# vita-epfl/collaborative-gan-sampling

Hardware: AMD Instinct MI355X
Metric: refined samples/sec @ 20 refinement steps (higher is better)
Workload: dtype f32; 1 GPU; dcgan64 collaborative refinement (propose + K-step refine + render), batch 1024/GPU, K=20, momentum rate 0.1, refine at feature [8, 8, 256], random-init weights, z~U(-1,1) seed 2019+rank; global_batch=1024, refine_steps=20, parallelism=single GPU, hipgraph=True, batches_in_flight=2, fused_per_launch=1, sync_bn=False, contraction=f32

## Files before the change

### collaborative-gan-sampling_amd/csrc/bn.hip

```cpp
#include "cgs_internal.h"

#define BN_MAX_BLOCKS CGS_BN_MAX_BLOCKS

struct BnGeom {
    int G;
    int rows_per_block;
};

static BnGeom bn_geom(int M, int C) {
    BnGeom g;
    int rpb = cgs_ceil_div(M, BN_MAX_BLOCKS);
    if (rpb < 16) rpb = 16;
    g.rows_per_block = rpb;
    g.G = cgs_ceil_div(M, rpb);
    (void)C;
    return g;
}

size_t cgs_bn_ws_bytes(int M, int C) {
    (void)M;
    return ((size_t)BN_MAX_BLOCKS * 2 * C + 6 * (size_t)C) * sizeof(float);
}

__device__ __forceinline__ void bn_affine4(const float* __restrict__ mean, const float* __restrict__ invstd, const float* __restrict__ gamma,
// ... 695 lines not shown
                                     const float* gamma, const float* beta, const float* mean, const float* invstd, float leak, float* dx,
                                     int M_group, int C, void* ws, size_t ws_bytes, void* stream) {
    if (groups <= 0 || groups > 65535 || M_group <= 0 || C <= 0 || (C & 3) || rows_per_seg <= 0 || nseg <= 0 || seg_stride < 0 || !part || !dy || !x || !dx)
        return cgs_set_error(CGS_EINVAL, "norm bwd from partials: groups=%d M=%d C=%d rows=%d x %d", groups, M_group, C, rows_per_seg, nseg);
    const bool sliced = groups == 1 && nseg == 1 && rows_per_seg >= 1024 && !((uintptr_t)ws & 7);
    const size_t need = (size_t)groups * 2 * C * sizeof(float) + (sliced ? (size_t)BNF_SLICES * 2 * C * sizeof(double) : 0);
    if (!ws || ws_bytes < need) return cgs_set_error(CGS_EWORKSPACE, "norm bwd from partials: workspace %zu < %zu", ws_bytes, need);
    hipStream_t s = (hipStream_t)stream;
    if (const int rpb = norm_fa_rows_per_block(groups, rows_per_seg, nseg, M_group, C)) {
        hipLaunchKernelGGL(norm_fa_kernel<true>, dim3(cgs_ceil_div(C, 64), cgs_ceil_div(M_group, rpb), groups), dim3(256), 0, s, x, dy, part, rows_per_seg, nseg,
                           seg_stride, gamma, beta, 0.f, leak, dx, (float*)mean, (float*)invstd, M_group, C, rpb);
        CGS_CHECK_LAUNCH("norm_lrelu_bwd_from_partials");
        return CGS_OK;
    }
    float* stat2;
    if (sliced) {
        double* slices = (double*)ws;
        stat2 = (float*)(slices + (size_t)BNF_SLICES * 2 * C);
        hipLaunchKernelGGL(bn_slice_sums_kernel, dim3(cgs_ceil_div(C, BNF_CH), BNF_SLICES), dim3(256), 0, s, part, rows_per_seg, C, slices);
        hipLaunchKernelGGL(bn_finalize2_slices_kernel, dim3(cgs_ceil_div(C, 64)), dim3(64), 0, s, slices, M_group, C, stat2);
    } else {
        stat2 = (float*)ws;
        hipLaunchKernelGGL(bn_finalize_kernel<1>, dim3(cgs_ceil_div(C, BNF_CH), groups), dim3(256), 0, s, part, rows_per_seg, M_group, C, nullptr, nullptr, 0.f,
                           stat2, nullptr, nullptr, nseg, seg_stride);
    }
    const size_t n4 = (size_t)groups * M_group * C / 4, gn4 = (size_t)M_group * C / 4;
    hipLaunchKernelGGL(bn_apply_bwd_kernel, dim3(ew_blocks(n4)), dim3(256), 0, s, dy, x, mean, invstd, gamma, beta, stat2, leak, dx, n4, C, gn4);
    CGS_CHECK_LAUNCH("norm_lrelu_bwd_from_partials");
    return CGS_OK;
}

int cgs_instnorm_lrelu_bwd_data(const float* dy, const float* x, const float* scale, const float* offset, const float* mean,
                                const float* invstd, float leak, float* dx, int B, int HW, int C, void* ws, size_t ws_bytes,
                                void* stream) {
    if (B <= 0 || HW <= 0 || C <= 0 || (C & 3) || B > 65535) return cgs_set_error(CGS_EINVAL, "instnorm bwd: B=%d HW=%d C=%d", B, HW, C);
    if (ws_bytes < cgs_instnorm_ws_bytes(B, HW, C)) return cgs_set_error(CGS_EWORKSPACE, "instnorm bwd: workspace %zu < %zu", ws_bytes, cgs_instnorm_ws_bytes(B, HW, C));
    hipStream_t s = (hipStream_t)stream;
    const BnGeom g = in_geom(B, HW);
    float* part = (float*)ws;
    float* stat = part + (size_t)B * g.G * 2 * C;
    float* stat2 = stat + (size_t)B * 4 * C;
    if (norm_small_ok(HW)) {
        hipLaunchKernelGGL(norm_small_kernel<true>, dim3(cgs_ceil_div(C, 64), B), dim3(256), 0, s, x, dy, scale, offset, 0.f, leak, dx, (float*)mean, (float*)invstd, stat2, HW, C);
        CGS_CHECK_LAUNCH("instnorm_lrelu_bwd_data");
        return CGS_OK;
    }
    hipLaunchKernelGGL(bn_partial_kernel<1>, dim3(g.G, B), dim3(256), 0, s, x, dy, mean, invstd, scale, offset, leak, part, HW, C, g.rows_per_block);
    hipLaunchKernelGGL(bn_finalize_kernel<1>, dim3(cgs_ceil_div(C, BNF_CH), B), dim3(256), 0, s, part, g.G, HW, C, nullptr, nullptr, 0.f, stat2, nullptr, nullptr);
    const size_t n4 = (size_t)B * HW * C / 4, gn4 = (size_t)HW * C / 4;
    hipLaunchKernelGGL(bn_apply_bwd_kernel, dim3(ew_blocks(n4)), dim3(256), 0, s, dy, x, mean, invstd, scale, offset, stat2, leak, dx, n4, C, gn4);
    CGS_CHECK_LAUNCH("instnorm_lrelu_bwd_data");
    return CGS_OK;
}
```

### collaborative-gan-sampling_amd/engine.py

```python
import gc

import numpy as np
import torch

from . import kernels as K
from . import lib as L
from .nets import ARCHS, _same_out, g_input_shape, layer_ks


class _Stage:
    out = None
    bwd_epi = (L.EPI_NONE, None, None)
    pre_folded = False
    bwd_nstat = None
    bstat = None

    def fwd(self, x):
        raise NotImplementedError

    def bwd(self, dy):
        raise NotImplementedError


class _View(_Stage):
# ... 47 lines not shown
            elif self.epi == L.EPI_TANH:
                dy = K.tanh_bwd(dy, self.out, out=dy)
        e, a, aux = self.bwd_epi
        return K.conv2d_bwd_data(dy, self.w, self.in_hw, self.s, self.s, out=self.dx, epilogue=e, ep_a=a, ep_aux=aux, nstat=self.bwd_nstat)


class _Deconv(_Stage):

    def __init__(self, B, in_shape, out_shape, w, b, stride, epi, a, c, dev):
        self.w, self.b, self.s, self.epi, self.a, self.c = w, b, stride, epi, a, c
        self.in_hw, self.out_hw = (in_shape[0], in_shape[1]), (out_shape[0], out_shape[1])
        self.out = torch.empty((B,) + tuple(out_shape), dtype=torch.float32, device=dev)
        self.dx = torch.empty((B,) + tuple(in_shape), dtype=torch.float32, device=dev)

    signs = None
    bwd_signs = None
    part = None
    part_layout = None

    def want_stats(self, B, group_images=None):
        if self.epi != L.EPI_NONE:
            return None
        lay = K.conv_stat_layout(L.DECONV_FWD, *self.call_dims(), self.s, self.s, group_images or B)
        if lay is not None:
            self.part = torch.empty((lay[0], 2, self.w.shape[2]), dtype=torch.float32, device=self.out.device)
            self.part_layout = lay
        return self.part

    def fwd(self, x):
        return K.deconv2d_fwd(x, self.w, self.b, self.out_hw, self.s, self.s, self.epi, self.a, self.c, out=self.out, signs=self.signs,
                              part=self.part)

    def bwd(self, dy):
        if not self.pre_folded:
            if self.epi == L.EPI_AFFINE_RELU:
                dy = K.affine_relu_bwd(dy, self.out, self.a, out=dy)
            elif self.epi == L.EPI_TANH:
                dy = K.tanh_bwd(dy, self.out, out=dy)
        e, a, aux = self.bwd_epi
        return K.deconv2d_bwd_data(dy, self.w, self.in_hw, self.s, self.s, out=self.dx, epilogue=e, ep_a=a, ep_aux=aux,
                                   ep_signs=self.bwd_signs, nstat=self.bwd_nstat)

    def call_dims(self):
        kh, kw, Cout, Cin = self.w.shape
        return (self.out.shape[0], self.in_hw[0], self.in_hw[1], Cin, self.out_hw[0], self.out_hw[1], Cout, kh, kw)


class _Linear(_Stage):
    def __init__(self, B, w, b, epi, dev):
        self.w, self.b, self.epi = w, b, epi
        self.out = torch.empty((B, w.shape[1]), dtype=torch.float32, device=dev)
        self.dx = torch.empty((B, w.shape[0]), dtype=torch.float32, device=dev)

    def fwd(self, x):
        self.x_in = x
        return K.linear_fwd(x, self.w, self.b, self.epi, out=self.out)

    def bwd(self, dy):
        if self.epi == L.EPI_LRELU:
            dy = K.lrelu_bwd(dy, self.out, out=dy)
        return K.linear_bwd_data(dy, self.w, out=self.dx)


class _BnTrainLrelu(_Stage):

    def __init__(self, B, shape, gamma, beta, leak, dev):
        self.gamma, self.beta, self.leak = gamma, beta, leak
        self.out = torch.empty((B,) + tuple(shape), dtype=torch.float32, device=dev)
        self.mean = torch.empty(shape[-1], dtype=torch.float32, device=dev)
        self.invstd = torch.empty(shape[-1], dtype=torch.float32, device=dev)
        self.x = None

    sync = None
    groups = 1
    part = None

    part_layout = None

    def set_groups(self, groups, producer=None):
        self.groups = int(groups)
        self.part = self.part_layout = None
        if producer is not None:
            producer.part = producer.part_layout = None
            B = self.out.shape[0]
            self.part = producer.want_stats(B, B // self.groups)
            self.part_layout = producer.part_layout
        C = self.out.shape[-1]
        self.mean = torch.empty((self.groups, C), dtype=torch.float32, device=self.out.device)
        self.invstd = torch.empty((self.groups, C), dtype=torch.float32, device=self.out.device)

    def _g(self, t):
        return t.view(self.groups, -1, t.shape[-1])

    def fwd(self, x):
        self.x = x
        if self.bstat is not None:
            self.bstat.x = x
        if self.groups > 1:
            if self.part is not None:
                K.groupnorm_lrelu_fwd_from_partials(x, self.part, self.part_layout, self.groups, self.gamma, self.beta, self.leak,
                                                    out=self.out, stats=(self.mean, self.invstd))
            else:
                K.instnorm_lrelu_fwd(self._g(x), self.gamma, self.beta, self.leak, out=self._g(self.out), stats=(self.mean, self.invstd))
            return self.out
        if self.sync is None:
            if self.part is not None:
                K.bn_train_lrelu_fwd_from_partials(x, self.part, self.gamma, self.beta, self.leak, out=self.out, stats=(self.mean, self.invstd))
            else:
                K.bn_train_lrelu_fwd(x, self.gamma, self.beta, self.leak, out=self.out, stats=(self.mean, self.invstd))
            return self.out
        M = x.numel() // x.shape[-1]
        sums = self.sync.sums(x.shape[-1], x.device)
        K.bn_sync_fwd_sums(x, sums)
        self.sync.all_reduce(sums)
        K.bn_sync_fwd_apply(x, self.gamma, self.beta, sums, self.sync.world * M, self.leak, out=self.out,
                            stats=(self.mean, self.invstd))
        return self.out

    def bwd(self, dy):
        if self.bstat is not None:
            return K.norm_lrelu_bwd_from_partials(dy, self.x, self.bstat, self.groups, out=dy)
        if self.groups > 1:
            K.instnorm_lrelu_bwd_data(self._g(dy), self._g(self.x), self.gamma, self.beta, self.mean, self.invstd, self.leak,
                                      out=self._g(dy))
            return dy
        if self.sync is None:
            return K.bn_train_lrelu_bwd_data(dy, self.x, self.gamma, self.beta, self.mean, self.invstd, self.leak, out=dy)
        M = self.x.numel() // self.x.shape[-1]
        sums = self.sync.sums(self.x.shape[-1], dy.device)
        K.bn_sync_bwd_sums(dy, self.x, self.gamma, self.beta, self.mean, self.invstd, sums, self.leak)
        self.sync.all_reduce(sums)
        return K.bn_sync_bwd_apply(dy, self.x, self.gamma, self.beta, self.mean, self.invstd, sums, self.sync.world * M,
                                   self.leak, out=dy)


class BnSync:

    def __init__(self, group=None):
        import torch.distributed as dist
        if not (dist.is_available() and dist.is_initialized()):
            raise L.CgsError("sync_bn needs an initialised torch.distributed process group")
        self.dist, self.group = dist, group
        self.world = dist.get_world_size(group)
        self.on_device = dist.get_backend(group) == "nccl"
        self._sums = {}

    def sums(self, C, dev):
        key = (C, dev)
        if key not in self._sums:
            self._sums[key] = torch.empty((2, C), dtype=torch.float64, device=dev)
        return self._sums[key]

    def all_reduce(self, sums):
        if self.world == 1:
            return
        if self.on_device:
            self.dist.all_reduce(sums, group=self.group)
        else:
            h = sums.cpu()
            self.dist.all_reduce(h, group=self.group)
            sums.copy_(h)


class _InstNormAct(_Stage):

    def __init__(self, B, shape, scale, offset, leak, dev):
        self.scale, self.offset, self.leak = scale, offset, leak
        self.out = torch.empty((B,) + tuple(shape), dtype=torch.float32, device=dev)
        self.mean = torch.empty((B, shape[-1]), dtype=torch.float32, device=dev)
        self.invstd = torch.empty((B, shape[-1]), dtype=torch.float32, device=dev)
        self.x = None

# ... 123 lines not shown
            else:
                if kind(i + 1) != "relu":
                    raise NotImplementedError("inference-mode bn is only supported when followed by relu")
                a, c = fold(Lr[1])
                stages.append(_AffineRelu(B, shape, a, c, dev)); i += 2
        elif t == "instnorm":
            sc = f"{scope}/{Lr[1]}"
            leak, used = (K.LEAK, 2) if kind(i + 1) == "lrelu" else (0.0, 2) if kind(i + 1) == "relu" else (1.0, 1)
            in_stage = _InstNormAct(B, shape, P[sc + "/scale"], P[sc + "/offset"], leak, dev)
            if stages and isinstance(stages[-1], (_Conv, _Deconv)):
                in_stage.part = stages[-1].want_stats(B, 1)
                in_stage.part_layout = stages[-1].part_layout
            stages.append(in_stage); i += used
        elif t == "res":
            inner, ishape = compile_layers(Lr[1], shape, P, scope, B, k, stride, bn_training, dev, folds)
            assert tuple(ishape) == tuple(shape)
            stages.append(_Residual(B, shape, inner, dev)); i += 1
        elif t in ("relu", "lrelu", "tanh"):
            stages.append(_Unary(B, shape, t, dev)); i += 1
        elif t == "reshape":
            stages.append(_View((B,) + shape, (B,) + tuple(Lr[1]))); shape = tuple(Lr[1]); i += 1
        elif t == "flatten":
            flat = (int(np.prod(shape)),)
            stages.append(_View((B,) + shape, (B,) + flat)); shape = flat; i += 1
        else:
            raise KeyError(t)
    return stages, shape


def link_backward_fusion(stages):
    for below, above in zip(stages[:-1], stages[1:]):
        if not isinstance(above, (_Conv, _Deconv)) or below.pre_folded:
            continue
        if isinstance(below, _Deconv) and below.epi == L.EPI_AFFINE_RELU:
            above.bwd_epi = (L.EPI_RELU_BWD_AFFINE, below.a, below.out)
            import os
            if isinstance(above, _Deconv) and not os.environ.get("CGS_NO_SIGN_MASKS"):
                s_ = (below.s, below.s)
                if (K.conv_signs_ok(L.DECONV_FWD, *below.call_dims(), *s_, L.EPI_AFFINE_RELU)
                        and K.conv_signs_ok(L.DECONV_BWD_DATA, *above.call_dims(), above.s, above.s, L.EPI_RELU_BWD_AFFINE)):
                    below.signs = torch.empty(below.out.numel() // 32, dtype=torch.int32, device=below.out.device)
                    above.bwd_signs = below.signs
        elif isinstance(below, _Deconv) and below.epi == L.EPI_TANH:
            above.bwd_epi = (L.EPI_TANH_BWD, None, below.out)
        elif isinstance(below, _Conv) and below.epi == L.EPI_LRELU:
            above.bwd_epi = (L.EPI_LRELU_BWD, None, below.out)
        elif isinstance(below, _Conv) and below.epi == L.EPI_TANH:
            above.bwd_epi = (L.EPI_TANH_BWD, None, below.out)
        else:
            continue
        below.pre_folded = True


NSTAT_MAX_BYTES = 48 * 2 ** 20


def link_norm_backward_stats(stages, B):
    for below, above in zip(stages[:-1], stages[1:]):
        if isinstance(below, _Residual):
            link_norm_backward_stats(below.inner, B)
        if not isinstance(above, (_Conv, _Deconv)) or above.bwd_epi[0] != L.EPI_NONE or above.bwd_nstat is not None:
            continue
        if isinstance(below, _BnTrainLrelu) and below.sync is None:
            gamma, beta, gimg = below.gamma, below.beta, B // below.groups
        elif isinstance(below, _InstNormAct):
            gamma, beta, gimg = below.scale, below.offset, 1
        else:
            continue
        C = below.out.shape[-1]
        if below.out.numel() * 4 > NSTAT_MAX_BYTES:
            continue
        if isinstance(above, _Conv):
            H, W, Cin = above.dx.shape[1:]
            kh, kw, _, Cout = above.w.shape
            lay = K.conv_stat_layout(L.CONV_BWD_DATA, B, H, W, Cin, 0, 0, Cout, kh, kw, above.s, above.s, gimg)
        else:
            lay = K.conv_stat_layout(L.DECONV_BWD_DATA, *above.call_dims(), above.s, above.s, gimg)
        if lay is None:
            continue
        part = torch.empty((lay[0], 2, C), dtype=torch.float32, device=below.out.device)
        below.bstat = above.bwd_nstat = K.NormBwdStats(None, below.mean, below.invstd, gamma, beta, below.leak, gimg, part, lay)
    if stages and isinstance(stages[-1], _Residual):
        link_norm_backward_stats(stages[-1].inner, B)


class Tape:

    def __init__(self, layers, in_shape, P, scope, B, k, stride, bn_training, dev):
        self.folds = []
        self.stages, self.out_shape = compile_layers(layers, in_shape, P, scope, B, k, stride, bn_training, dev, self.folds)

    def forward(self, x):
        for st in self.stages:
            x = st.fwd(x)
        return x

    def backward(self, dy):
        for st in reversed(self.stages):
            dy = st.bwd(dy)
        return dy


def _entry(fn):
    import functools

    @functools.wraps(fn)
    def wrapped(self, *a, **kw):
        prev = K.set_contraction(self.contraction)
        try:
            return fn(self, *a, **kw)
        finally:
            if prev != self.contraction:
                K.set_contraction(prev)
    return wrapped


class RefineEngine:

    def __init__(self, arch, params, batch_size, device=None, use_graph=False, sync_bn=None, bn_groups=1, contraction="f32"):
        self.A = ARCHS[arch] if isinstance(arch, str) else arch
        if contraction not in L.CONTRACTIONS:
            raise L.CgsError(f"contraction {contraction!r}: expected one of {sorted(L.CONTRACTIONS)}")
        self.contraction = contraction
        self.dev = torch.device(device if device is not None else "cuda:0")
        if self.dev.type != "cuda":
            raise L.CgsError("RefineEngine needs a GPU device (there is no CPU path)")
        L.load()
        prev_mode = K.set_contraction(self.contraction)
        try:
            self._build(params, batch_size, use_graph, sync_bn, bn_groups)
        finally:
            if prev_mode != self.contraction:
                K.set_contraction(prev_mode)

    def _build(self, params, batch_size, use_graph, sync_bn, bn_groups):
        A, B = self.A, int(batch_size)
        self.B, self.P = B, params
        with torch.cuda.device(self.dev):
            self.g_head = Tape(A["g_head"], g_input_shape(A), params, "generator", B, A["k"], A["stride"], False, self.dev)
            self.g_tail = Tape(A["g_tail"], A["feature"], params, "generator", B, A["k"], A["stride"], False, self.dev)
            self.d = Tape(A["d"], A["img"], params, "discriminator", B, A["k"], A["stride"], True, self.dev)
            link_backward_fusion(self.g_tail.stages + self.d.stages)
            fs = (B,) + tuple(A["feature"])
            f32 = dict(dtype=torch.float32, device=self.dev)
            self.theta, self.mom, self.best_theta = torch.empty(fs, **f32), torch.empty(fs, **f32), torch.empty(fs, **f32)
            self.logit, self.best_logit = torch.empty(B, **f32), torch.empty(B, **f32)
            self.default_logit, self.best_step = torch.empty(B, **f32), torch.empty(B, **f32)
            self.tickets = torch.zeros(B, dtype=torch.int32, device=self.dev)
            self.dlogits = torch.empty((B,) + tuple(self.d.out_shape), **f32)
            self.forced = torch.zeros(B, dtype=torch.int32, device=self.dev)
            self.images = torch.empty((B,) + tuple(A["img"]), **f32)
        self.use_graph = use_graph
        self._graphs = {}
        self._gstream = None
        self._ws_epoch = K.WS.epoch
        self.bn_groups = int(bn_groups)
        if self.bn_groups > 1:
            if B % self.bn_groups:
                raise L.CgsError(f"bn_groups={bn_groups} does not divide the engine batch {B}")
            if sync_bn:
                raise L.CgsError("bn_groups and sync_bn are mutually exclusive")

            def walk_g(stages):
                for below, st in zip([None] + stages[:-1], stages):
                    if isinstance(st, _BnTrainLrelu):
                        st.set_groups(self.bn_groups, below if isinstance(below, _Conv) else None)
                    if isinstance(st, _Residual):
                        walk_g(st.inner)
            walk_g(self.d.stages); walk_g(self.g_tail.stages)
        self.sync_bn = None
        if sync_bn is not None and sync_bn is not False:
            if use_graph:
                raise L.CgsError("sync_bn runs eagerly: the all-reduce between the two halves of a bn pass is not captured")
            self.sync_bn = BnSync(None if sync_bn is True else sync_bn)

            def walk(stages):
                for st in stages:
                    if isinstance(st, _BnTrainLrelu):
                        st.sync = self.sync_bn
                    if isinstance(st, _Residual):
                        walk(st.inner)
            walk(self.d.stages); walk(self.g_tail.stages)

        def drop_partials(stages):
            for below, st in zip([None] + stages[:-1], stages):
                if isinstance(st, _BnTrainLrelu) and st.sync is not None:
                    st.part = None
                    if isinstance(below, _Conv):
                        below.part = None
                if isinstance(st, _Residual):
                    drop_partials(st.inner)
        drop_partials(self.d.stages); drop_partials(self.g_tail.stages)
        link_norm_backward_stats(self.g_tail.stages + self.d.stages, B)

    def _sync_weights(self):
        if self._ws_epoch != K.WS.epoch:
            self._resync()

    def _resync(self):
        K.set_contraction(self.contraction)
        epoch = K.WS.epoch
        with torch.cuda.device(self.dev):
            for tape in (self.g_head, self.g_tail, self.d):
                for a, c, gamma, beta, mm, mv in tape.folds:
                    K.bn_fold(gamma, beta, mm, mv, out=(a, c))
            if self._gstream is not None and self._graphs:
                cur = torch.cuda.current_stream(self.dev)
                self._gstream.wait_stream(cur)
                with torch.cuda.stream(self._gstream):
                    self.forward_logits(self.theta, self.logit)
                    self.backward_to_feature()
                cur.wait_stream(self._gstream)
        self._ws_epoch = epoch

    @_entry
    def input_to_feature(self, z):
        self._sync_weights()
        return self.g_head.forward(z)

    @_entry
    def feature_to_data(self, feat):
        self._sync_weights()
        return self.g_tail.forward(feat)

    @_entry
    def discriminator(self, x):
        self._sync_weights()
        return self.d.forward(x)

    @_entry
    def generate(self, z):
        self._sync_weights()
        return self.g_tail.forward(self.g_head.forward(z))

    @_entry
    def score(self, images, out=None):
        self._sync_weights()
        return K.sigmoid_rowmean(self.d.forward(images), out=out)

    def forward_logits(self, theta, logit_out):
        x = self.g_tail.forward(theta)
        head = self.d.stages[-1]
        if isinstance(head, _Linear) and head.w.shape[1] == 1 and head.epi == L.EPI_NONE:
            for st in self.d.stages[:-1]:
                x = st.fwd(x)
            head.x_in = x
# ... 96 lines not shown
```

### collaborative-gan-sampling_amd/kernels.py

```python
import math
import weakref

import torch

from . import lib as L

LEAK = 0.2
BN_EPS = 1e-5


def _chk(t, name):
    if not (isinstance(t, torch.Tensor) and t.is_cuda and t.dtype == torch.float32 and t.is_contiguous()):
        raise L.CgsError(f"{name}: expected a contiguous fp32 tensor on the GPU, got "
                         f"{type(t).__name__} {getattr(t, 'dtype', None)} {getattr(t, 'device', None)}")
    return t


def _ptr(t):
    return None if t is None else t.data_ptr()


def _stream():
    return torch.cuda.current_stream().cuda_stream

# ... 427 lines not shown
    key = (B, HW, C, device.index, torch.cuda.current_stream(device).cuda_stream)
    ws = _in_ws.get(key)
    if ws is None:
        ws = torch.empty(int(L.load().cgs_instnorm_ws_bytes(B, HW, C)) // 4 + 4, dtype=torch.float32, device=device)
        _in_ws[key] = ws
    return ws


def instnorm_lrelu_fwd(x, scale, offset, leak=1.0, eps=BN_EPS, out=None, stats=None):
    _chk(x, "x")
    B, C = x.shape[0], x.shape[-1]
    HW = x.numel() // (B * C)
    y = out if out is not None else torch.empty_like(x)
    mean, invstd = stats if stats is not None else (torch.empty((B, C), dtype=torch.float32, device=x.device),
                                                     torch.empty((B, C), dtype=torch.float32, device=x.device))
    ws = _in_workspace(B, HW, C, x.device)
    pr = _Prof(0.0, "", _nb(x, x, y), op="instnorm_lrelu_fwd") if PROFILE is not None else None
    L.call("cgs_instnorm_lrelu_fwd", _ptr(x), _ptr(scale), _ptr(offset), eps, leak, _ptr(y), _ptr(mean), _ptr(invstd), B, HW, C,
           _ptr(ws), ws.numel() * 4, _stream())
    if pr is not None:
        pr.done()
    return y, mean, invstd


def instnorm_lrelu_bwd_data(dy, x, scale, offset, mean, invstd, leak=1.0, out=None):
    _chk(dy, "dy"); _chk(x, "x")
    B, C = x.shape[0], x.shape[-1]
    HW = x.numel() // (B * C)
    dx = out if out is not None else torch.empty_like(x)
    ws = _in_workspace(B, HW, C, x.device)
    pr = _Prof(0.0, "", _nb(dy, x, dy, x, dx), op="instnorm_lrelu_bwd_data") if PROFILE is not None else None
    L.call("cgs_instnorm_lrelu_bwd_data", _ptr(dy), _ptr(x), _ptr(scale), _ptr(offset), _ptr(mean), _ptr(invstd), leak, _ptr(dx),
           B, HW, C, _ptr(ws), ws.numel() * 4, _stream())
    if pr is not None:
        pr.done()
    return dx


def norm_lrelu_bwd_from_partials(dy, x, nstat, groups, out=None):
    _chk(dy, "dy"); _chk(x, "x")
    C_ = x.shape[-1]
    Mg = x.numel() // (groups * C_)
    dx = out if out is not None else torch.empty_like(x)
    ws = _in_workspace(groups, Mg, C_, x.device) if groups > 1 else _bn_workspace(Mg, C_, x.device)
    lay = nstat.layout
    pr = _Prof(0.0, "", _nb(dy, x, dx), op="norm_lrelu_bwd_from_partials") if PROFILE is not None else None
    L.call("cgs_norm_lrelu_bwd_from_partials", _ptr(dy), _ptr(x), _ptr(nstat.part), groups, lay[1], lay[2], lay[3], _ptr(nstat.gamma), _ptr(nstat.beta),
           _ptr(nstat.mean), _ptr(nstat.invstd), nstat.leak, _ptr(dx), Mg, C_, _ptr(ws), ws.numel() * 4, _stream())
    if pr is not None:
        pr.done()
    return dx


def add(a, b, out=None):
    _chk(a, "a"); _chk(b, "b")
    o = out if out is not None else torch.empty_like(a)
    L.call("cgs_add", _ptr(a), _ptr(b), _ptr(o), a.numel(), _stream())
    return o


def bn_fold(gamma, beta, moving_mean, moving_var, eps=BN_EPS, out=None):
    C = gamma.numel()
    a, b = out if out is not None else (torch.empty(C, dtype=torch.float32, device=gamma.device),
                                        torch.empty(C, dtype=torch.float32, device=gamma.device))
    L.call("cgs_bn_fold", _ptr(gamma), _ptr(beta), _ptr(moving_mean), _ptr(moving_var), eps, _ptr(a), _ptr(b), C, _stream())
    return a, b


def affine_relu_fwd(x, a, b, out=None):
    _chk(x, "x")
    C = x.shape[-1]
    y = out if out is not None else torch.empty_like(x)
    L.call("cgs_affine_relu_fwd", _ptr(x), _ptr(a), _ptr(b), _ptr(y), x.numel() // C, C, _stream())
    return y


def affine_relu_bwd(dy, y, a, out=None):
    _chk(dy, "dy"); _chk(y, "y")
    C = y.shape[-1]
    dx = out if out is not None else torch.empty_like(y)
    L.call("cgs_affine_relu_bwd", _ptr(dy), _ptr(y), _ptr(a), _ptr(dx), y.numel() // C, C, _stream())
    return dx


def affine_fwd(x, a, b, out=None):
    _chk(x, "x")
    C = x.shape[-1]
    y = out if out is not None else torch.empty_like(x)
    L.call("cgs_affine_fwd", _ptr(x), _ptr(a), _ptr(b), _ptr(y), x.numel() // C, C, _stream())
    return y


def affine_bwd(dy, a, out=None):
    _chk(dy, "dy")
    C = dy.shape[-1]
    dx = out if out is not None else torch.empty_like(dy)
    L.call("cgs_affine_bwd", _ptr(dy), _ptr(a), _ptr(dx), dy.numel() // C, C, _stream())
    return dx


def lrelu_fwd(x, leak=LEAK, out=None):
    _chk(x, "x")
    y = out if out is not None else torch.empty_like(x)
    L.call("cgs_lrelu_fwd", _ptr(x), leak, _ptr(y), x.numel(), _stream())
    return y

# ... 170 lines not shown
```

### collaborative-gan-sampling_amd/lib.py

```python
import ctypes as C
import os

_HERE = os.path.dirname(os.path.abspath(__file__))
LIB_PATH = os.environ.get("CGS_LIB") or os.path.join(_HERE, "libcgs_hip.so")

OK, EINVAL, EWORKSPACE, ELAUNCH = 0, -1, -2, -3
EPI_NONE, EPI_LRELU, EPI_AFFINE_RELU, EPI_TANH = 0, 1, 2, 3
EPI_RELU_BWD_AFFINE, EPI_LRELU_BWD, EPI_TANH_BWD = 4, 5, 6
CONV_FWD, CONV_BWD_DATA, DECONV_FWD, DECONV_BWD_DATA = 0, 1, 2, 3
FAMILY_IGEMM, FAMILY_QUAD, FAMILY_SMALLN_T, FAMILY_SMALLN_F, FAMILY_PATCH, FAMILY_TAPS, FAMILY_DOT, FAMILY_IGEMM_BX6 = 0, 1, 2, 3, 4, 5, 6, 7
CONTRACTION_F32, CONTRACTION_BX6, CONTRACTION_BX6_ALL = 0, 1, 2
CONTRACTIONS = {"f32": CONTRACTION_F32, "bx6": CONTRACTION_BX6, "bx6_all": CONTRACTION_BX6_ALL}

_p, _i, _f, _z = C.c_void_p, C.c_int, C.c_float, C.c_size_t
_ll = C.c_longlong

SIGNATURES = {
    "cgs_version": (_i, []),
    "cgs_source_sha": (C.c_char_p, []),
    "cgs_last_error": (C.c_char_p, []),
    "cgs_last_kernel": (C.c_char_p, []),
    "cgs_last_executed_flops": (C.c_double, []),
    "cgs_last_tail_tiles": (_i, []),
    "cgs_last_tail_split": (_i, []),
    "cgs_set_contraction": (_i, [_i]),
    "cgs_get_contraction": (_i, []),
    "cgs_conv_ws_bytes": (_z, [_i] * 7),
    "cgs_conv_ws_bytes_for": (_z, [_i] * 10),
    "cgs_conv_family": (_i, [_i] * 13 + [_z]),
    "cgs_conv2d_nhwc_fwd": (_i, [_p] * 4 + [_i] * 9 + [_i, _p, _p, _p, _z, _i, _p]),
    "cgs_conv_stat_partials": (_i, [_i] * 9 + [_z]),
    "cgs_conv2d_nhwc_fwd_stats": (_i, [_p] * 4 + [_i] * 9 + [_p, _z, _i, _p, _z, _p]),
    "cgs_conv_stat_layout": (_i, [_i] * 13 + [_z, _p, _p, _p]),
    "cgs_deconv2d_nhwc_fwd_stats": (_i, [_p] * 4 + [_i] * 11 + [_p, _z, _i, _p, _z, _p]),
    "cgs_conv2d_nhwc_bwd_data_nstats": (_i, [_p] * 3 + [_i] * 9 + [_p] * 5 + [_f, _i, _p, _z, _i, _p, _z, _p]),
    "cgs_deconv2d_nhwc_bwd_data_nstats": (_i, [_p] * 3 + [_i] * 11 + [_p] * 5 + [_f, _i, _p, _z, _i, _p, _z, _p]),
    "cgs_norm_lrelu_bwd_from_partials": (_i, [_p] * 3 + [_i] * 4 + [_p] * 4 + [_f, _p, _i, _i, _p, _z, _p]),
    "cgs_groupnorm_lrelu_fwd_from_partials": (_i, [_p, _p, _i, _i, _i, _i, _p, _p, _f, _f, _p, _p, _p, _i, _i, _p, _z, _p]),
    "cgs_bn_train_lrelu_fwd_from_partials": (_i, [_p, _p, _i, _p, _p, _f, _f, _p, _p, _p, _i, _i, _p, _z, _p]),
    "cgs_conv2d_nhwc_bwd_data": (_i, [_p] * 3 + [_i] * 9 + [_i, _p, _p, _p, _z, _i, _p]),
    "cgs_deconv2d_nhwc_fwd": (_i, [_p] * 4 + [_i] * 11 + [_i, _p, _p, _p, _z, _i, _p]),
    "cgs_deconv2d_nhwc_bwd_data": (_i, [_p] * 3 + [_i] * 11 + [_i, _p, _p, _p, _z, _i, _p]),
    "cgs_conv_signs_ok": (_i, [_i] * 13 + [_z]),
    "cgs_deconv2d_nhwc_fwd_signs": (_i, [_p] * 4 + [_i] * 11 + [_i, _p, _p, _p, _p, _z, _i, _p]),
    "cgs_deconv2d_nhwc_bwd_data_signs": (_i, [_p] * 3 + [_i] * 11 + [_i, _p, _p, _p, _z, _i, _p]),
    "cgs_linear_fwd": (_i, [_p] * 4 + [_i] * 4 + [_p, _z, _i, _p]),
    "cgs_linear_bwd_data": (_i, [_p] * 3 + [_i] * 3 + [_p, _z, _i, _p]),
    "cgs_bn_ws_bytes": (_z, [_i, _i]),
    "cgs_bn_train_lrelu_fwd": (_i, [_p, _p, _p, _f, _f, _p, _p, _p, _i, _i, _p, _z, _p]),
    "cgs_bn_train_lrelu_bwd_data": (_i, [_p] * 6 + [_f, _p, _i, _i, _p, _z, _p]),
    "cgs_bn_sync_fwd_sums": (_i, [_p, _p, _i, _i, _p, _z, _p]),
    "cgs_bn_sync_fwd_apply": (_i, [_p, _p, _p, _f, _f, _p, _ll, _p, _p, _p, _i, _i, _p, _z, _p]),
    "cgs_bn_sync_bwd_sums": (_i, [_p] * 6 + [_f, _p, _i, _i, _p, _z, _p]),
    "cgs_bn_sync_bwd_apply": (_i, [_p] * 6 + [_f, _p, _ll, _p, _i, _i, _p, _z, _p]),
    "cgs_instnorm_ws_bytes": (_z, [_i, _i, _i]),
    "cgs_instnorm_lrelu_fwd": (_i, [_p, _p, _p, _f, _f, _p, _p, _p, _i, _i, _i, _p, _z, _p]),
    "cgs_instnorm_lrelu_bwd_data": (_i, [_p] * 6 + [_f, _p, _i, _i, _i, _p, _z, _p]),
    "cgs_add": (_i, [_p, _p, _p, _z, _p]),
    "cgs_bn_fold": (_i, [_p] * 4 + [_f, _p, _p, _i, _p]),
    "cgs_affine_relu_fwd": (_i, [_p] * 4 + [_i, _i, _p]),
    "cgs_affine_relu_bwd": (_i, [_p] * 4 + [_i, _i, _p]),
    "cgs_affine_fwd": (_i, [_p] * 4 + [_i, _i, _p]),
    "cgs_affine_bwd": (_i, [_p] * 3 + [_i, _i, _p]),
    "cgs_lrelu_fwd": (_i, [_p, _f, _p, _z, _p]),
    "cgs_lrelu_bwd": (_i, [_p, _p, _f, _p, _z, _p]),
    "cgs_tanh_fwd": (_i, [_p, _p, _z, _p]),
    "cgs_tanh_bwd": (_i, [_p, _p, _p, _z, _p]),
    "cgs_bce_ones_grad_rowmean": (_i, [_p, _p, _p, _i, _i, _p]),
    "cgs_bce_ones_fwd": (_i, [_p, _p, _z, _p]),
    "cgs_bce_ones_bwd": (_i, [_p, _p, _p, _z, _p]),
    "cgs_sigmoid_rowmean": (_i, [_p, _p, _i, _i, _p]),
    "cgs_clip": (_i, [_p, _f, _f, _p, _z, _p]),
    "cgs_refine_update": (_i, [_p, _p, _p, _f, _f, _i, _i, _f, _f, _z, _p]),
    "cgs_refine_select": (_i, [_p, _p, _p, _i, _p, _p, _p, _i, _i, _p]),
    "cgs_refine_select_rows": (_i, [_p, _p, _p, _i, _p, _p, _i, _i, _p]),
    "cgs_refine_select2": (_i, [_p, _p, _i, _p, _p, _i, _p, _p, _i, _p, _p, _p, _i, _p]),
    "cgs_linear_out1_bce": (_i, [_p, _p, _p, _p, _p, _p, _i, _i, _p]),
    "cgs_mlp2d_sigmoid_saliency": (_i, [_p, _p, _i, _i, _p, _p, _p, _i, _f, _p]),
    "cgs_refine2d": (_i, [_p, _p, _i, _i, _p, _f, _f, _i, _f, _i, _p, _p, _p, _i, _p]),
    "cgs_refine2d_devbase": (_i, [_p, _p, _i, _i, _p, _p, _f, _i, _f, _i, _p, _p, _p, _i, _p]),
    "cgs_mlp2d_train_ws_bytes": (_z, [_i, _i]),
    "cgs_mlp2d_d_step": (_i, [_p, _p, _i, _i, _p, _i, _p, _i, _f, _p, _p, _p, _p, _z, _p]),
    "cgs_mlp2d_wide_train_ws_bytes": (_z, [_i, _i, _i]),
    "cgs_mlp2d_wide_d_step": (_i, [_p, _p, _i, _i, _p, _i, _p, _i, _f, _p, _p, _p, _p, _z, _p]),
    "cgs_mlp2d_gen_ws_bytes": (_z, [_i, _i, _i]),
    "cgs_mlp2d_gen_fwd": (_i, [_p] * 6 + [_i, _i, _p, _p, _i, _i, _f, _p, _p, _z, _p]),
    "cgs_mlp2d_wide_gen_ws_bytes": (_z, [_i, _i, _i]),
    "cgs_mlp2d_wide_gen_fwd": (_i, [_p] * 6 + [_i, _i, _p, _p, _i, _i, _f, _p, _p, _z, _p]),
    "cgs_mlp2d_g_step": (_i, [_p] * 6 + [_i, _i, _p, _p, _i, _f, _f, _p, _p, _p, _p, _z, _p]),
    "cgs_conv_wgrad_ws_bytes": (_z, [_i] * 9),
    "cgs_conv2d_nhwc_bwd_weight": (_i, [_p] * 3 + [_i] * 9 + [_i, _p, _z, _p]),
    "cgs_linear_bwd_weight": (_i, [_p] * 3 + [_i] * 3 + [_i, _p, _z, _p]),
    "cgs_bias_grad": (_i, [_p, _p, _i, _i, _i, _p, _z, _p]),
    "cgs_bn_train_param_grads": (_i, [_p, _i, _i, _p, _p, _i, _p]),
    "cgs_bce_logits_grad": (_i, [_p, _f, _f, _p, _p, _i, _p]),
    "cgs_adam_step": (_i, [_p, _p, _p, _p, _f, _f, _f, _f, _z, _p]),
}

_lib = None
stale = None


class CgsError(RuntimeError):
# ... 97 lines not shown
```

### include/cgs_hip.h

```cpp
#ifndef CGS_HIP_H
#define CGS_HIP_H

#include <stddef.h>
#include <stdint.h>

#ifdef __cplusplus
extern "C" {
#endif

#define CGS_OK 0
#define CGS_EINVAL (-1)
#define CGS_EWORKSPACE (-2)
#define CGS_ELAUNCH (-3)

#define CGS_EPI_NONE 0
#define CGS_EPI_LRELU 1
#define CGS_EPI_AFFINE_RELU 2
#define CGS_EPI_TANH 3
#define CGS_EPI_RELU_BWD_AFFINE 4
#define CGS_EPI_LRELU_BWD 5
#define CGS_EPI_TANH_BWD 6

#define CGS_CONV_FWD 0
#define CGS_CONV_BWD_DATA 1
// ... 54 lines not shown
int cgs_deconv2d_nhwc_bwd_data_nstats(const float* dy, const float* w, float* dx,
                                      int B, int H, int W, int Cin, int Ho, int Wo, int Cout, int kh, int kw, int sh, int sw,
                                      const float* x_norm, const float* mean, const float* invstd, const float* gamma, const float* beta,
                                      float leak, int group_images, void* ws, size_t ws_bytes, int ws_prepacked,
                                      float* stat_part, size_t stat_part_bytes, void* stream);
int cgs_norm_lrelu_bwd_from_partials(const float* dy, const float* x, const float* part, int groups, int rows_per_seg, int nseg,
                                     int seg_stride, const float* gamma, const float* beta, const float* mean, const float* invstd,
                                     float leak, float* dx, int M_group, int C, void* ws, size_t ws_bytes, void* stream);

int cgs_conv2d_nhwc_bwd_data(const float* dy, const float* w, float* dx,
                             int B, int H, int W, int Cin, int Cout, int kh, int kw, int sh, int sw,
                             int epilogue, const float* ep_a, const float* ep_aux,
                             void* ws, size_t ws_bytes, int ws_prepacked, void* stream);

int cgs_deconv2d_nhwc_fwd(const float* x, const float* w, const float* bias, float* y,
                          int B, int H, int W, int Cin, int Ho, int Wo, int Cout, int kh, int kw, int sh, int sw,
                          int epilogue, const float* ep_a, const float* ep_b,
                          void* ws, size_t ws_bytes, int ws_prepacked, void* stream);

int cgs_deconv2d_nhwc_bwd_data(const float* dy, const float* w, float* dx,
                               int B, int H, int W, int Cin, int Ho, int Wo, int Cout, int kh, int kw, int sh, int sw,
                               int epilogue, const float* ep_a, const float* ep_aux,
                               void* ws, size_t ws_bytes, int ws_prepacked, void* stream);

int cgs_conv_signs_ok(int op, int B, int H, int W, int Cin, int Ho, int Wo, int Cout, int kh, int kw, int sh, int sw,
                      int epilogue, size_t ws_bytes);
int cgs_deconv2d_nhwc_fwd_signs(const float* x, const float* w, const float* bias, float* y,
                                int B, int H, int W, int Cin, int Ho, int Wo, int Cout, int kh, int kw, int sh, int sw,
                                int epilogue, const float* ep_a, const float* ep_b, unsigned* signs,
                                void* ws, size_t ws_bytes, int ws_prepacked, void* stream);
int cgs_deconv2d_nhwc_bwd_data_signs(const float* dy, const float* w, float* dx,
                                     int B, int H, int W, int Cin, int Ho, int Wo, int Cout, int kh, int kw, int sh, int sw,
                                     int epilogue, const float* ep_a, const unsigned* aux_signs,
                                     void* ws, size_t ws_bytes, int ws_prepacked, void* stream);

int cgs_linear_fwd(const float* x, const float* w, const float* bias, float* y, int B, int in, int out,
                   int epilogue, void* ws, size_t ws_bytes, int ws_prepacked, void* stream);
int cgs_linear_out1_bce(const float* x, const float* w, const float* bias, float* logits, float* dlogits, float* logit_mean, int B, int in,
                        void* stream);
int cgs_linear_bwd_data(const float* dy, const float* w, float* dx, int B, int in, int out,
                        void* ws, size_t ws_bytes, int ws_prepacked, void* stream);

size_t cgs_bn_ws_bytes(int M, int C);
int cgs_bn_train_lrelu_fwd(const float* x, const float* gamma, const float* beta, float eps, float leak,
                           float* y, float* mean, float* invstd, int M, int C,
                           void* ws, size_t ws_bytes, void* stream);
int cgs_bn_train_lrelu_fwd_from_partials(const float* x, const float* part, int G, const float* gamma, const float* beta,
                                         float eps, float leak, float* y, float* mean, float* invstd, int M, int C,
                                         void* ws, size_t ws_bytes, void* stream);
int cgs_bn_train_lrelu_bwd_data(const float* dy, const float* x, const float* gamma, const float* beta,
                                const float* mean, const float* invstd, float leak, float* dx, int M, int C,
                                void* ws, size_t ws_bytes, void* stream);

int cgs_bn_sync_fwd_sums(const float* x, double* sums, int M, int C, void* ws, size_t ws_bytes, void* stream);
int cgs_bn_sync_fwd_apply(const float* x, const float* gamma, const float* beta, float eps, float leak, const double* sums,
                          long long M_total, float* y, float* mean, float* invstd, int M, int C,
                          void* ws, size_t ws_bytes, void* stream);
int cgs_bn_sync_bwd_sums(const float* dy, const float* x, const float* gamma, const float* beta, const float* mean,
                         const float* invstd, float leak, double* sums, int M, int C, void* ws, size_t ws_bytes, void* stream);
int cgs_bn_sync_bwd_apply(const float* dy, const float* x, const float* gamma, const float* beta, const float* mean,
                          const float* invstd, float leak, const double* sums, long long M_total, float* dx, int M, int C,
                          void* ws, size_t ws_bytes, void* stream);

size_t cgs_instnorm_ws_bytes(int B, int HW, int C);
int cgs_instnorm_lrelu_fwd(const float* x, const float* scale, const float* offset, float eps, float leak, float* y,
                           float* mean, float* invstd, int B, int HW, int C, void* ws, size_t ws_bytes, void* stream);
int cgs_instnorm_lrelu_bwd_data(const float* dy, const float* x, const float* scale, const float* offset,
                                const float* mean, const float* invstd, float leak, float* dx, int B, int HW, int C,
                                void* ws, size_t ws_bytes, void* stream);
int cgs_groupnorm_lrelu_fwd_from_partials(const float* x, const float* part, int groups, int rows_per_seg, int nseg, int seg_stride,
                                          const float* gamma, const float* beta, float eps, float leak, float* y, float* mean,
                                          float* invstd, int M_group, int C, void* ws, size_t ws_bytes, void* stream);
int cgs_add(const float* a, const float* b, float* out, size_t n, void* stream);

int cgs_bn_fold(const float* gamma, const float* beta, const float* moving_mean, const float* moving_var,
                float eps, float* a, float* b, int C, void* stream);
int cgs_affine_relu_fwd(const float* x, const float* a, const float* b, float* y, int M, int C, void* stream);
int cgs_affine_relu_bwd(const float* dy, const float* y, const float* a, float* dx, int M, int C, void* stream);
int cgs_affine_fwd(const float* x, const float* a, const float* b, float* y, int M, int C, void* stream);
int cgs_affine_bwd(const float* dy, const float* a, float* dx, int M, int C, void* stream);
int cgs_lrelu_fwd(const float* x, float leak, float* y, size_t n, void* stream);
int cgs_lrelu_bwd(const float* dy, const float* y, float leak, float* dx, size_t n, void* stream);
int cgs_tanh_fwd(const float* x, float* y, size_t n, void* stream);
int cgs_tanh_bwd(const float* dy, const float* y, float* dx, size_t n, void* stream);

int cgs_bce_ones_grad_rowmean(const float* logits, float* dlogits, float* logit_mean, int B, int P, void* stream);

int cgs_bce_ones_fwd(const float* logits, float* loss, size_t n, void* stream);
int cgs_bce_ones_bwd(const float* dloss, const float* logits, float* dlogits, size_t n, void* stream);
int cgs_sigmoid_rowmean(const float* logits, float* sigmoids, int B, int P, void* stream);
int cgs_clip(const float* x, float vmin, float vmax, float* y, size_t n, void* stream);

int cgs_refine_update(float* theta, float* m, const float* g, float rate, float alpha, int first,
                      int use_clip, float vmin, float vmax, size_t n, void* stream);
int cgs_refine_select(const float* theta, const float* logit, const int32_t* forced, int step_index,
                      float* best_theta, float* best_logit, float* best_step, int B, int F, void* stream);
int cgs_refine_select2(const float* rows, float* best_rows, int Frows, const float* theta, float* best_theta, int F, const float* logit,
                       const int32_t* forced, int step_index, float* best_logit, float* best_step, int* tickets, int B, void* stream);
int cgs_refine_select_rows(const float* src, const float* logit, const int32_t* forced, int step_index, float* dst,
                           const float* best_logit, int B, int F, void* stream);

int cgs_mlp2d_sigmoid_saliency(const float* const* w, const float* const* b, int nlayers, int nhidden, const float* x,
                               float* sigmoid, float* saliency, int B, float inv_batch, void* stream);
int cgs_refine2d(const float* const* w, const float* const* b, int nlayers, int nhidden, const float* x,
                 float real_sigmoid_mean, float inv_batch, int steps, float rate, int method,
                 float* best_x, float* best_step, float* traj, int B, void* stream);
// ... 43 lines not shown
```

Baseline: 6434 samples/s.

## Fuse final linear backward into the norm-lrelu backward under the discriminator head

When a single-output linear head sits directly on a batch/instance norm + leaky-ReLU stage, the head's backward is skipped and the norm backward rebuilds dy on the fly as dlogit[b]*w[p,c] inside its partial-reduction and apply kernels. This removes the materialised dy tensor write and read plus a separate linear backward launch. It also removes the size cap on precomputed backward norm statistics, so those links apply to larger layers too. In exchange it adds coupling between stages and new kernels with extra index arithmetic.

```diff
diff --git a/collaborative-gan-sampling_amd/csrc/bn.hip b/collaborative-gan-sampling_amd/csrc/bn.hip
--- a/collaborative-gan-sampling_amd/csrc/bn.hip
+++ b/collaborative-gan-sampling_amd/csrc/bn.hip
@@ -771,3 +771,150 @@
     CGS_CHECK_LAUNCH("instnorm_lrelu_bwd_data");
     return CGS_OK;
 }
+
+__device__ __forceinline__ float4 ul_dy4(float dl, const float4 w) {
+#pragma clang fp contract(off)
+    return make_float4(dl * w.x, dl * w.y, dl * w.z, dl * w.w);
+}
+
+__global__ __launch_bounds__(256) void bn_partial_ul_kernel(const float* __restrict__ x, const float* __restrict__ dl, const float* __restrict__ w,
+                                                            const float* __restrict__ mean_p, const float* __restrict__ invstd_p ,
+                                                            const float* __restrict__ gamma, const float* __restrict__ beta,
+                                                            float leak, float* __restrict__ part, int M, int C, int HW,
+                                                            int rows_per_block) {
+    __shared__ float4 red[2][256];
+    x += (size_t)blockIdx.y * M * C;
+    dl += (size_t)blockIdx.y * (M / HW);
+    mean_p += (size_t)blockIdx.y * C; invstd_p += (size_t)blockIdx.y * C;
+    part += (size_t)blockIdx.y * gridDim.x * 2 * C;
+    const int tid = threadIdx.x;
+    const int r0 = blockIdx.x * rows_per_block;
+    const int r1 = min(M, r0 + rows_per_block);
+    const int CQ = C >> 2;
+    int tpr = 1;
+    while (tpr * 2 <= CQ && tpr * 2 <= 256) tpr *= 2;
+    const int rg = tid / tpr, RG = 256 / tpr, tc = tid - rg * tpr;
+    const int step_b = RG / HW, step_p = RG - step_b * HW;
+    for (int q0 = 0; q0 < CQ; q0 += tpr) {
+        const int cq = q0 + tc;
+        float4 sa = make_float4(0.f, 0.f, 0.f, 0.f), sb = sa;
+        if (cq < CQ) {
+            float4 mean, invstd, scale, shift;
+            bn_affine4(mean_p, invstd_p, gamma, beta, 4 * cq, mean, invstd, scale, shift);
+            int b = (r0 + rg) / HW, p = (r0 + rg) - b * HW;
+            for (int r = r0 + rg; r < r1; r += RG) {
+                const float4 xv = ((const float4*)(x + (size_t)r * C))[cq];
+                const float4 dv = ul_dy4(dl[b], ((const float4*)(w + (size_t)p * C))[cq]);
+#define P1(f)                                                                   \
+                {                                                               \
+                    const float u = fmaf(xv.f, scale.f, shift.f);               \
+                    const float d = dv.f * (u > 0.f ? 1.f : leak);              \
+                    sa.f += d; sb.f = fmaf(d, (xv.f - mean.f) * invstd.f, sb.f); \
+                }
+                P1(x) P1(y) P1(z) P1(w)
+#undef P1
+                b += step_b; p += step_p;
+                if (p >= HW) { p -= HW; ++b; }
+            }
+        }
+        red[0][tid] = sa; red[1][tid] = sb;
+        __syncthreads();
+        if (rg == 0 && cq < CQ) {
+            float4 ta = make_float4(0.f, 0.f, 0.f, 0.f), tb = ta;
+            for (int gq = 0; gq < RG; ++gq) {
+                const float4 a = red[0][gq * tpr + tc], b = red[1][gq * tpr + tc];
+                ta.x += a.x; ta.y += a.y; ta.z += a.z; ta.w += a.w;
+                tb.x += b.x; tb.y += b.y; tb.z += b.z; tb.w += b.w;
+            }
+            ((float4*)(part + ((size_t)blockIdx.x * 2 + 0) * C))[cq] = ta;
+            ((float4*)(part + ((size_t)blockIdx.x * 2 + 1) * C))[cq] = tb;
+        }
+        __syncthreads();
+    }
+}
+
+#define BWD1(f)                                                       \
+        {                                                             \
+            const float u = fmaf(xv.f, sc.f, sh.f);                   \
+            const float d = dv.f * (u > 0.f ? 1.f : leak);            \
+            const float xh = (xv.f - mean.f) * inv.f;                 \
+            o.f = sc.f * (d - m1.f - xh * m2.f);                      \
+        }
+__global__ __launch_bounds__(256) void bn_apply_bwd_ul_kernel(const float* __restrict__ dl, const float* __restrict__ w, const float* __restrict__ x,
+                                                              const float* __restrict__ mean0, const float* __restrict__ invstd0,
+                                                              const float* __restrict__ gamma, const float* __restrict__ beta,
+                                                              const float* __restrict__ stat20,
+                                                              float leak, float* __restrict__ dx, size_t n4, int C, size_t group_n4, size_t K4) {
+    const size_t stride = (size_t)gridDim.x * blockDim.x;
+    size_t i = (size_t)blockIdx.x * blockDim.x + threadIdx.x;
+    if (i >= n4) return;
+    if (((stride * 4) % (size_t)C) == 0) {
+        const int c = (int)((i * 4) % C);
+        size_t grp = i / group_n4, grp_end = (grp + 1) * group_n4;
+        size_t b = i / K4, k4 = i - b * K4;
+        const size_t step_b = stride / K4, step_k = stride - step_b * K4;
+        float4 mean, inv, sc, sh, m1, m2;
+        bn_affine4(mean0 + grp * C, invstd0 + grp * C, gamma, beta, c, mean, inv, sc, sh);
+        m1 = *(const float4*)(stat20 + grp * 2 * C + c); m2 = *(const float4*)(stat20 + grp * 2 * C + C + c);
+        for (; i < n4; i += stride) {
+            if (i >= grp_end) {
+                grp = i / group_n4; grp_end = (grp + 1) * group_n4;
+                bn_affine4(mean0 + grp * C, invstd0 + grp * C, gamma, beta, c, mean, inv, sc, sh);
+                m1 = *(const float4*)(stat20 + grp * 2 * C + c); m2 = *(const float4*)(stat20 + grp * 2 * C + C + c);
+            }
+            const float4 xv = ((const float4*)x)[i], dv = ul_dy4(dl[b], ((const float4*)w)[k4]);
+            float4 o;
+            BWD1(x) BWD1(y) BWD1(z) BWD1(w)
+            ((float4*)dx)[i] = o;
+            b += step_b; k4 += step_k;
+            if (k4 >= K4) { k4 -= K4; ++b; }
+        }
+        return;
+    }
+    for (; i < n4; i += stride) {
+        const size_t grp = i / group_n4;
+        const float* stat2 = stat20 + grp * 2 * C;
+        const int c = (int)((i * 4) % C);
+        const size_t b = i / K4;
+        const float4 xv = ((const float4*)x)[i], dv = ul_dy4(dl[b], ((const float4*)w)[i - b * K4]);
+        float4 mean, inv, sc, sh;
+        bn_affine4(mean0 + grp * C, invstd0 + grp * C, gamma, beta, c, mean, inv, sc, sh);
+        const float4 m1 = *(const float4*)(stat2 + c), m2 = *(const float4*)(stat2 + C + c);
+        float4 o;
+        BWD1(x) BWD1(y) BWD1(z) BWD1(w)
+        ((float4*)dx)[i] = o;
+    }
+}
+#undef BWD1
+
+int cgs_norm_lrelu_bwd_under_linear(const float* dlogit, const float* w, const float* x, const float* gamma, const float* beta, const float* mean,
+                                    const float* invstd, float leak, float* dx, int groups, int M_group, int HW, int C, void* ws, size_t ws_bytes,
+                                    void* stream) {
+    if (groups <= 0 || groups > 65535 || M_group <= 0 || HW <= 0 || M_group % HW || C <= 0 || (C & 3) || !dlogit || !w || !x || !dx)
+        return cgs_set_error(CGS_EINVAL, "norm bwd under linear: groups=%d M=%d HW=%d C=%d (M must be whole samples of HW rows, C a multiple of 4)", groups,
+                             M_group, HW, C);
+    const size_t need = groups > 1 ? cgs_instnorm_ws_bytes(groups, M_group, C) : cgs_bn_ws_bytes(M_group, C);
+    if (!ws || ws_bytes < need) return cgs_set_error(CGS_EWORKSPACE, "norm bwd under linear: workspace %zu < %zu", ws_bytes, need);
+    if ((long long)groups * M_group > 0x7fffffffLL) return cgs_set_error(CGS_EINVAL, "norm bwd under linear: %d x %d rows", groups, M_group);
+    hipStream_t s = (hipStream_t)stream;
+    const BnGeom g = groups > 1 ? in_geom(groups, M_group) : bn_geom(M_group, C);
+    float* part = (float*)ws;
+    float* stat = part + (groups > 1 ? (size_t)groups * g.G * 2 * C : (size_t)BN_MAX_BLOCKS * 2 * C);
+    float* stat2 = stat + (size_t)groups * 4 * C;
+    if (norm_small_ok(M_group)) {
+        if (int rc = cgs_linear_bwd_data(dlogit, w, dx, groups * (M_group / HW), HW * C, 1, nullptr, 0, 0, stream)) return rc;
+        hipLaunchKernelGGL(norm_small_kernel<true>, dim3(cgs_ceil_div(C, 64), groups), dim3(256), 0, s, x, dx, gamma, beta, 0.f, leak, dx, (float*)mean,
+                           (float*)invstd, stat2, M_group, C);
+        CGS_CHECK_LAUNCH("norm_lrelu_bwd_under_linear");
+        return CGS_OK;
+    }
+    hipLaunchKernelGGL(bn_partial_ul_kernel, dim3(g.G, groups), dim3(256), 0, s, x, dlogit, w, mean, invstd, gamma, beta, leak, part, M_group, C, HW,
+                       g.rows_per_block);
+    hipLaunchKernelGGL(bn_finalize_kernel<1>, dim3(cgs_ceil_div(C, BNF_CH), groups), dim3(256), 0, s, part, g.G, M_group, C, nullptr, nullptr, 0.f, stat2, nullptr,
+                       nullptr);
+    const size_t n4 = (size_t)groups * M_group * C / 4, gn4 = (size_t)M_group * C / 4;
+    hipLaunchKernelGGL(bn_apply_bwd_ul_kernel, dim3(ew_blocks(n4)), dim3(256), 0, s, dlogit, w, x, mean, invstd, gamma, beta, stat2, leak, dx, n4, C, gn4,
+                       (size_t)HW * C / 4);
+    CGS_CHECK_LAUNCH("norm_lrelu_bwd_under_linear");
+    return CGS_OK;
+}
diff --git a/collaborative-gan-sampling_amd/engine.py b/collaborative-gan-sampling_amd/engine.py
--- a/collaborative-gan-sampling_amd/engine.py
+++ b/collaborative-gan-sampling_amd/engine.py
@@ -123,11 +123,16 @@
         self.out = torch.empty((B, w.shape[1]), dtype=torch.float32, device=dev)
         self.dx = torch.empty((B, w.shape[0]), dtype=torch.float32, device=dev)
 
+    norm_below = None
+
     def fwd(self, x):
         self.x_in = x
         return K.linear_fwd(x, self.w, self.b, self.epi, out=self.out)
 
     def bwd(self, dy):
+        if self.norm_below is not None:
+            self.norm_below.dlogit = dy
+            return self.dx
         if self.epi == L.EPI_LRELU:
             dy = K.lrelu_bwd(dy, self.out, out=dy)
         return K.linear_bwd_data(dy, self.w, out=self.dx)
@@ -147,6 +152,8 @@
     part = None
 
     part_layout = None
+    head = None
+    dlogit = None
 
     def set_groups(self, groups, producer=None):
         self.groups = int(groups)
@@ -189,6 +196,10 @@
         return self.out
 
     def bwd(self, dy):
+        if self.head is not None:
+            K.norm_lrelu_bwd_under_linear(self.dlogit, self.head.w, self.x, self.gamma, self.beta, self.mean, self.invstd, self.leak,
+                                          self.groups, out=dy.view(self.x.shape))
+            return dy
         if self.bstat is not None:
             return K.norm_lrelu_bwd_from_partials(dy, self.x, self.bstat, self.groups, out=dy)
         if self.groups > 1:
@@ -418,7 +429,16 @@
         below.pre_folded = True
 
 
-NSTAT_MAX_BYTES = 48 * 2 ** 20
+def link_norm_under_linear(stages):
+    for i, head in enumerate(stages):
+        if not (isinstance(head, _Linear) and head.w.shape[1] == 1 and head.epi == L.EPI_NONE):
+            continue
+        j = i - 1
+        if j >= 0 and isinstance(stages[j], _View):
+            j -= 1
+        below = stages[j] if j >= 0 else None
+        if isinstance(below, _BnTrainLrelu) and below.sync is None and below.bstat is None:
+            below.head, head.norm_below = head, below
 
 
 def link_norm_backward_stats(stages, B):
@@ -434,8 +454,6 @@
         else:
             continue
         C = below.out.shape[-1]
-        if below.out.numel() * 4 > NSTAT_MAX_BYTES:
-            continue
         if isinstance(above, _Conv):
             H, W, Cin = above.dx.shape[1:]
             kh, kw, _, Cout = above.w.shape
@@ -483,11 +501,13 @@
 
 class RefineEngine:
 
-    def __init__(self, arch, params, batch_size, device=None, use_graph=False, sync_bn=None, bn_groups=1, contraction="f32"):
+    def __init__(self, arch, params, batch_size, device=None, use_graph=False, sync_bn=None, bn_groups=1, contraction="f32",
+                 fused_norm_backward=True):
         self.A = ARCHS[arch] if isinstance(arch, str) else arch
         if contraction not in L.CONTRACTIONS:
             raise L.CgsError(f"contraction {contraction!r}: expected one of {sorted(L.CONTRACTIONS)}")
         self.contraction = contraction
+        self.fused_norm_backward = bool(fused_norm_backward)
         self.dev = torch.device(device if device is not None else "cuda:0")
         if self.dev.type != "cuda":
             raise L.CgsError("RefineEngine needs a GPU device (there is no CPU path)")
@@ -557,7 +577,9 @@
                 if isinstance(st, _Residual):
                     drop_partials(st.inner)
         drop_partials(self.d.stages); drop_partials(self.g_tail.stages)
-        link_norm_backward_stats(self.g_tail.stages + self.d.stages, B)
+        if self.fused_norm_backward:
+            link_norm_backward_stats(self.g_tail.stages + self.d.stages, B)
+            link_norm_under_linear(self.d.stages)
 
     def _sync_weights(self):
         if self._ws_epoch != K.WS.epoch:
diff --git a/collaborative-gan-sampling_amd/kernels.py b/collaborative-gan-sampling_amd/kernels.py
--- a/collaborative-gan-sampling_amd/kernels.py
+++ b/collaborative-gan-sampling_amd/kernels.py
@@ -503,6 +503,23 @@
     return dx
 
 
+def norm_lrelu_bwd_under_linear(dlogit, w, x, gamma, beta, mean, invstd, leak=LEAK, groups=1, out=None):
+    _chk(dlogit, "dlogit"); _chk(w, "w"); _chk(x, "x")
+    B, C_ = x.shape[0], x.shape[-1]
+    HW = x.numel() // (B * C_)
+    if dlogit.numel() != B or w.numel() != HW * C_ or B % groups:
+        raise L.CgsError(f"norm_lrelu_bwd_under_linear: x {tuple(x.shape)}, dlogit {tuple(dlogit.shape)}, w {tuple(w.shape)}, groups {groups}")
+    Mg = (B // groups) * HW
+    dx = out if out is not None else torch.empty_like(x)
+    ws = _in_workspace(groups, Mg, C_, x.device) if groups > 1 else _bn_workspace(Mg, C_, x.device)
+    pr = _Prof(0.0, "", _nb(x, x, dx), op="norm_lrelu_bwd_under_linear") if PROFILE is not None else None
+    L.call("cgs_norm_lrelu_bwd_under_linear", _ptr(dlogit), _ptr(w), _ptr(x), _ptr(gamma), _ptr(beta), _ptr(mean), _ptr(invstd), leak,
+           _ptr(dx), groups, Mg, HW, C_, _ptr(ws), ws.numel() * 4, _stream())
+    if pr is not None:
+        pr.done()
+    return dx
+
+
 def add(a, b, out=None):
     _chk(a, "a"); _chk(b, "b")
     o = out if out is not None else torch.empty_like(a)
diff --git a/collaborative-gan-sampling_amd/lib.py b/collaborative-gan-sampling_amd/lib.py
--- a/collaborative-gan-sampling_amd/lib.py
+++ b/collaborative-gan-sampling_amd/lib.py
@@ -49,6 +49,7 @@
     "cgs_bn_ws_bytes": (_z, [_i, _i]),
     "cgs_bn_train_lrelu_fwd": (_i, [_p, _p, _p, _f, _f, _p, _p, _p, _i, _i, _p, _z, _p]),
     "cgs_bn_train_lrelu_bwd_data": (_i, [_p] * 6 + [_f, _p, _i, _i, _p, _z, _p]),
+    "cgs_norm_lrelu_bwd_under_linear": (_i, [_p] * 7 + [_f, _p, _i, _i, _i, _i, _p, _z, _p]),
     "cgs_bn_sync_fwd_sums": (_i, [_p, _p, _i, _i, _p, _z, _p]),
     "cgs_bn_sync_fwd_apply": (_i, [_p, _p, _p, _f, _f, _p, _ll, _p, _p, _p, _i, _i, _p, _z, _p]),
     "cgs_bn_sync_bwd_sums": (_i, [_p] * 6 + [_f, _p, _i, _i, _p, _z, _p]),
diff --git a/include/cgs_hip.h b/include/cgs_hip.h
--- a/include/cgs_hip.h
+++ b/include/cgs_hip.h
@@ -130,6 +130,10 @@
                                 const float* mean, const float* invstd, float leak, float* dx, int M, int C,
                                 void* ws, size_t ws_bytes, void* stream);
 
+int cgs_norm_lrelu_bwd_under_linear(const float* dlogit, const float* w, const float* x, const float* gamma, const float* beta,
+                                    const float* mean, const float* invstd, float leak, float* dx, int groups, int M_group, int HW,
+                                    int C, void* ws, size_t ws_bytes, void* stream);
+
 int cgs_bn_sync_fwd_sums(const float* x, double* sums, int M, int C, void* ws, size_t ws_bytes, void* stream);
 int cgs_bn_sync_fwd_apply(const float* x, const float* gamma, const float* beta, float eps, float leak, const double* sums,
                           long long M_total, float* y, float* mean, float* invstd, int M, int C,
```

Measured after the change: 6464 samples/s, median of 6. No clear change (+0.5%).
